# cyh-0/CAVP

Hardware: AMD Instinct MI355X
Metric: frames/sec end-to-end CAVP fwd+bwd, B=32 224x224 (higher is better)
Workload: dtype bf16; 1 GPU; C1' (config_avss_binary shape): CAVP ResNet-50 OS16 + VGGish, training step = forward_train (batch-stat BN, 32 images + 64 audio clips per GPU) + cross-entropy + full backward, 224x224 RGB + 96x64 mel, num_classes=2, random-init (synthetic) weights; global_batch=32, per_gpu_batch=32, parallelism=dp1, ranks=1, launch=hipGraph replay, deterministic=False

## Files before the change

cavp_amd/csrc/conv_igemm_big.hip:

```cpp
#include <type_traits>

#include "igemm_params.h"

#define CAVP_USE8(a) asm volatile("" : "+v"(a[0]), "+v"(a[1]), "+v"(a[2]), "+v"(a[3]), "+v"(a[4]), "+v"(a[5]), "+v"(a[6]), "+v"(a[7]))

namespace {

constexpr int BC = 256, BP = 256, NT = 512;
constexpr int HALF_BYTES = 128 * 128;
constexpr int BUF_BYTES = 4 * HALF_BYTES;
constexpr int RING_BYTES = 2 * BUF_BYTES;
constexpr int SCR_BYTES = 4096;
constexpr int LDS_BYTES = RING_BYTES + 8 * SCR_BYTES;
constexpr unsigned kOOB = 0x80000000u;
static_assert(LDS_BYTES == 160 * 1024, "the whole LDS of a CU");

typedef __attribute__((address_space(3))) void* lds_ptr_t;

}

template <int DBG>
__global__ __launch_bounds__(512, 2) void igemm_big_kernel(const IgemmParams p) {
  extern __shared__ __attribute__((aligned(16))) char smem[];
  cavp_prefetch_kernargs<(int)sizeof(IgemmParams)>();
  const int tid = threadIdx.x, lane = tid & 63;
  const int wave = __builtin_amdgcn_readfirstlane(tid >> 6);
  const int wc = wave & 3, wp = wave >> 2;
  const int lrow = lane & 15, lgrp = lane >> 4;

  const __amdgpu_buffer_rsrc_t xrsrc = __builtin_amdgcn_make_buffer_rsrc((void*)p.x, 0, p.x_bytes, 0x00020000);
  const __amdgpu_buffer_rsrc_t wrsrc = __builtin_amdgcn_make_buffer_rsrc((void*)p.w, 0, p.w_bytes, 0x00020000);

  const int my_tiles = ((int)blockIdx.x < p.nblk) ? (p.nblk - 1 - (int)blockIdx.x) / (int)gridDim.x + 1 : 0;
  if (my_tiles == 0) return;
  const int HoWo = p.Ho * p.Wo;

  const int r0 = 8 * wave + (lane >> 3);
  const int kslot = ((lane & 7) ^ ((4 * wave + (lane >> 4)) & 7)) * 8;
  const int kbyte = kslot * 2;
  unsigned w_off[4];
  unsigned x_off[4];
  unsigned x_mask[4];
  int iss_tile = 0;
  int iss_ti = 0, iss_cc = 0;
  int iss_buf = 0;
  int iss_woff = p.tap_woff[0], iss_xoff = p.tap_xoff[0];

  auto setup_tile = [&](int ord) {
    const int vb = (int)blockIdx.x + ord * (int)gridDim.x;
    const int sid = xcd_remap(vb, p.nblk);
    const int tp = fast_div(sid, p.div_tc_m, p.div_tc_s), tc = sid - tp * p.tiles_c;
    const int c_base = tc * BC, p_base = tp * BP;
#pragma unroll
    for (int m = 0; m < 4; ++m) {
      const int r = r0 + 64 * (m & 1), half = m >> 1;
      const int c = c_base + (r >> 5) * 64 + half * 32 + (r & 31);
      w_off[m] = c < p.Cout ? (unsigned)(((size_t)c * p.K + kslot) * 2) : kOOB;
    }
    int h0[4], w0[4];
#pragma unroll
    for (int m = 0; m < 4; ++m) {
      const int r = r0 + 64 * (m & 1), half = m >> 1;
      const int pix = p_base + (r >> 6) * 128 + half * 64 + (r & 63);
      const bool ok = pix < p.M;
      const int pp = ok ? pix : 0;
      const int n = fast_div(pp, p.div_hw_m, p.div_hw_s), rr = pp - n * HoWo;
      const int ho = fast_div(rr, p.div_w_m, p.div_w_s), wo = rr - ho * p.Wo;
      h0[m] = ok ? ho * p.stride - p.pad : -0x10000000;
      w0[m] = wo * p.stride_w - p.pad;
      x_mask[m] = 0;
      x_off[m] = (unsigned)((n * p.H + h0[m]) * p.W + w0[m]) * (unsigned)(p.ldx * 2) + (unsigned)kbyte;
    }
    for (int t = 0; t < p.ntaps; ++t) {
      const int dh = p.tap_dh[t], dw = p.tap_dw[t];
#pragma unroll
      for (int m = 0; m < 4; ++m)
        x_mask[m] |= ((unsigned)(h0[m] + dh) < (unsigned)p.H && (unsigned)(w0[m] + dw) < (unsigned)p.W) ? (1u << t) : 0u;
    }
  };

  auto issue_half = [&](auto kc) {
    constexpr int K = decltype(kc)::value;
    const bool live = iss_tile < my_tiles;
    const int ti = iss_ti, c0 = iss_cc * 64;
    const unsigned oobm = (live && (c0 + kslot) < p.Cin) ? 0u : kOOB;
    char* base = smem + iss_buf * BUF_BYTES + K * HALF_BYTES + wave * 1024;
    if constexpr ((DBG & 8) != 0) {
    } else if constexpr ((K & 1) == 0) {
      const unsigned wk = (unsigned)(iss_woff + c0 * 2);
#pragma unroll
      for (int j = 0; j < 2; ++j) {
        const unsigned off = (w_off[(K >> 1) * 2 + j] + wk) | oobm;
        __builtin_amdgcn_raw_ptr_buffer_load_lds(wrsrc, (lds_ptr_t)(base + j * 8192), 16, (int)off, 0, 0, 0);
      }
    } else {
      const unsigned xk = (unsigned)(iss_xoff + c0 * 2);
#pragma unroll
      for (int j = 0; j < 2; ++j) {
        const int m = (K >> 1) * 2 + j;
        const unsigned tapm = ((~(x_mask[m] >> ti)) & 1u) << 31;
        __builtin_amdgcn_raw_ptr_buffer_load_lds(xrsrc, (lds_ptr_t)(base + j * 8192), 16, (int)((x_off[m] + xk) | tapm | oobm), 0, 0,
                                                 0);
      }
    }
    if constexpr (K == 3) {
      iss_buf ^= 1;
      if (live) {
        if constexpr ((DBG & 1) != 0) {
          if (++iss_cc == p.cpt) {
            iss_cc = 0;
            if (++iss_ti == p.ntaps) {
              iss_ti = 0;
              if (++iss_tile < my_tiles) setup_tile(iss_tile);
            }
            iss_woff = p.tap_woff[iss_ti];
            iss_xoff = p.tap_xoff[iss_ti];
          }
        } else {
          if (++iss_ti == p.ntaps) {
            iss_ti = 0;
            if (++iss_cc == p.cpt) {
              iss_cc = 0;
              if (++iss_tile < my_tiles) setup_tile(iss_tile);
            }
          }
          iss_woff = p.tap_woff[iss_ti];
          iss_xoff = p.tap_xoff[iss_ti];
        }
      }
    }
  };

  f32x4_t acc[4][8];
#pragma unroll
  for (int a = 0; a < 4; ++a)
#pragma unroll
    for (int b = 0; b < 8; ++b) acc[a][b] = (f32x4_t){0.f, 0.f, 0.f, 0.f};
  u32x4_t fa0[2][2], fa1[2][2], fb[4][2];

  const int key = (lrow >> 1) & 7;
  const int a_off = (wc * 32 + lrow) * 128 + ((lgrp ^ key) << 4);
  const int b_off = (wp * 64 + lrow) * 128 + ((lgrp ^ key) << 4);
  int cmp_buf = 0, cmp_k = 0, cmp_tile = 0;

  auto read_a = [&](u32x4_t (&f)[2][2], int half) {
    const char* base = smem + cmp_buf * BUF_BYTES + (half ? 2 : 0) * HALF_BYTES + a_off;
#pragma unroll
    for (int a = 0; a < 2; ++a) {
      f[a][0] = *(const u32x4_t*)(base + a * 2048);
      f[a][1] = *(const u32x4_t*)(base + a * 2048 + ((((lgrp ^ key) ^ 4) - (lgrp ^ key)) << 4));
    }
  };
  auto read_b = [&](int half) {
    const char* base = smem + cmp_buf * BUF_BYTES + (half ? 3 : 1) * HALF_BYTES + b_off;
#pragma unroll
    for (int b = 0; b < 4; ++b) {
      fb[b][0] = *(const u32x4_t*)(base + b * 2048);
      fb[b][1] = *(const u32x4_t*)(base + b * 2048 + ((((lgrp ^ key) ^ 4) - (lgrp ^ key)) << 4));
    }
  };
  auto mma_quadrant = [&](const u32x4_t (&f)[2][2], auto hc, auto hq) {
    constexpr int HC = decltype(hc)::value, HQ = decltype(hq)::value;
#pragma unroll
    for (int j = 0; j < 2; ++j)
#pragma unroll
      for (int a = 0; a < 2; ++a)
#pragma unroll
        for (int b = 0; b < 4; ++b) Mma<bf16_t>::run(acc[HC * 2 + a][HQ * 4 + b], f[a][j], fb[b][j]);
  };

  auto epilogue = [&](int ord) {
    const int vb = (int)blockIdx.x + ord * (int)gridDim.x;
    const int sid = xcd_remap(vb, p.nblk);
    const int tp = fast_div(sid, p.div_tc_m, p.div_tc_s), tc = sid - tp * p.tiles_c;
    const int c_wave = tc * BC + wc * 64, p_wave = tp * BP + wp * 128;
    const int nvw = p.M - p_wave;
    if (p.tile_stats) {
#pragma unroll
      for (int a = 0; a < 4; ++a) {
        float s1[4], s2[4], x0[4];
#pragma unroll
        for (int i = 0; i < 4; ++i) {
          x0[i] = row16_first(acc[a][0][i]);
          s1[i] = 0.f; s2[i] = 0.f;
        }
#pragma unroll
        for (int b = 0; b < 8; ++b) {
          const bool ok = b * 16 + lrow < nvw;
#pragma unroll
          for (int i = 0; i < 4; ++i) {
            const float d = ok ? acc[a][b][i] - x0[i] : 0.f;
            s1[i] += d;
            s2[i] = fmaf(d, d, s2[i]);
          }
        }
#pragma unroll
        for (int i = 0; i < 4; ++i) {
          s1[i] = row16_sum(s1[i]);
          s2[i] = row16_sum(s2[i]);
        }
        const int c = c_wave + a * 16 + lgrp * 4;
        if (lrow == 0 && nvw > 0 && c < p.Cout) {
          const float inv_n = fast_rcp((float)(nvw < 128 ? nvw : 128));
          float4 o;
          float m = s1[0] * inv_n; o.x = x0[0] + m; o.y = fmaxf(s2[0] - s1[0] * m, 0.f);
          m = s1[1] * inv_n; o.z = x0[1] + m; o.w = fmaxf(s2[1] - s1[1] * m, 0.f);
          float4 o2;
          m = s1[2] * inv_n; o2.x = x0[2] + m; o2.y = fmaxf(s2[2] - s1[2] * m, 0.f);
          m = s1[3] * inv_n; o2.z = x0[3] + m; o2.w = fmaxf(s2[3] - s1[3] * m, 0.f);
          float* dst = p.tile_stats + ((size_t)(tp * 2 + wp) * p.Cout + c) * 2;
          *(float4*)dst = o;
          *(float4*)(dst + 4) = o2;
        }
      }
    }
    float* scr = (float*)(smem + RING_BYTES + wave * SCR_BYTES);
    const int cg = lane & 7, ec = c_wave + cg * 8, pr = lane >> 3;
    const bool ec_ok = ec < p.Cout;
    float sc[8], sh[8];
#pragma unroll
    for (int e = 0; e < 8; ++e) { sc[e] = 1.f; sh[e] = 0.f; }
    if (ec_ok) {
      if (p.scale) {
#pragma unroll
        for (int q = 0; q < 2; ++q) {
          const float4 t = *(const float4*)(p.scale + ec + 4 * q);
          sc[4 * q] = t.x; sc[4 * q + 1] = t.y; sc[4 * q + 2] = t.z; sc[4 * q + 3] = t.w;
        }
        CAVP_USE8(sc);
      }
      if (p.shift) {
#pragma unroll
        for (int q = 0; q < 2; ++q) {
          const float4 t = *(const float4*)(p.shift + ec + 4 * q);
          sh[4 * q] = t.x; sh[4 * q + 1] = t.y; sh[4 * q + 2] = t.z; sh[4 * q + 3] = t.w;
        }
        CAVP_USE8(sh);
      }
    }
    const bool has_ss = p.scale != nullptr || p.shift != nullptr;
    bf16_t* yp = (bf16_t*)p.y + (size_t)(p_wave + pr) * p.ldy + ec;
    const bf16_t* rp = p.res ? (const bf16_t*)p.res + (size_t)((p.res_rows ? p_wave % p.res_rows : p_wave) + pr) * p.ldr + ec : nullptr;
    bf16_t* xp = p.aux_mode ? (bf16_t*)p.aux + (size_t)(p_wave + pr) * p.ld_aux + ec : nullptr;
#pragma unroll
    for (int b = 0; b < 8; ++b) {
      u32x4_t rr[2], mm[2];
      if (p.aux_mode == 2) {
#pragma unroll
        for (int k = 0; k < 2; ++k) {
          mm[k] = (u32x4_t){0u, 0u, 0u, 0u};
          if (ec_ok && b * 16 + pr + 8 * k < nvw) {
            mm[k] = *(const u32x4_t*)(xp + (size_t)(b * 16 + 8 * k) * p.ld_aux);
            asm volatile("" : "+v"(mm[k]));
          }
        }
      }
      if (rp) {
#pragma unroll
        for (int k = 0; k < 2; ++k) {
          rr[k] = (u32x4_t){0u, 0u, 0u, 0u};
          if (ec_ok && b * 16 + pr + 8 * k < nvw) {
            rr[k] = *(const u32x4_t*)(rp + (size_t)(b * 16 + 8 * k) * p.ldr);
            asm volatile("" : "+v"(rr[k]));
          }
        }
      }
#pragma unroll
      for (int a = 0; a < 4; ++a) *(f32x4_t*)(scr + lrow * 64 + (((a * 4 + lgrp) ^ lrow) << 2)) = acc[a][b];
      __builtin_amdgcn_s_waitcnt(0xc07f);
#pragma unroll
      for (int k = 0; k < 2; ++k) {
        const int px = pr + 8 * k;
        float v[8];
        {
          const f32x4_t t0 = *(const f32x4_t*)(scr + px * 64 + (((2 * cg) ^ px) << 2));
          const f32x4_t t1 = *(const f32x4_t*)(scr + px * 64 + (((2 * cg + 1) ^ px) << 2));
          v[0] = t0[0]; v[1] = t0[1]; v[2] = t0[2]; v[3] = t0[3];
          v[4] = t1[0]; v[5] = t1[1]; v[6] = t1[2]; v[7] = t1[3];
        }
        const int row = b * 16 + px;
        if (!(ec_ok && row < nvw)) continue;
        if (p.nbias) {
          const float* nb = p.nbias + (size_t)fast_div(p_wave + row, p.div_hw_m, p.div_hw_s) * p.Cout + ec;
          float nbv[8];
#pragma unroll
          for (int e = 0; e < 8; ++e) nbv[e] = nb[e];
          CAVP_USE8(nbv);
#pragma unroll
          for (int e = 0; e < 8; ++e) v[e] += nbv[e];
        }
        if (has_ss) {
#pragma unroll
          for (int e = 0; e < 8; ++e) v[e] = __fadd_rn(__fmul_rn(v[e], sc[e]), sh[e]);
        }
        if (p.aux_mode == 2) {
#pragma unroll
          for (int e = 0; e < 4; ++e) {
            v[2 * e] *= __uint_as_float(mm[k][e] << 16);
            v[2 * e + 1] *= __uint_as_float(mm[k][e] & 0xffff0000u);
          }
        }
        if (rp) {
#pragma unroll
          for (int e = 0; e < 4; ++e) {
            v[2 * e] += __uint_as_float(rr[k][e] << 16);
            v[2 * e + 1] += __uint_as_float(rr[k][e] & 0xffff0000u);
          }
        }
        if (p.aux_mode == 1) {
          float dgv[8];
#pragma unroll
          for (int e = 0; e < 8; ++e) gelu_and_grad(v[e], v[e], dgv[e]);
          u32x4_t d;
#pragma unroll
          for (int e = 0; e < 4; ++e) d[e] = pack2bf(dgv[2 * e], dgv[2 * e + 1]);
          __builtin_nontemporal_store(d, (u32x4_t*)(xp + (size_t)(b * 16 + 8 * k) * p.ld_aux));
        } else {
          apply_act_vec<8, true>(v, p.act);
        }
        u32x4_t o;
#pragma unroll
        for (int e = 0; e < 4; ++e) o[e] = pack2bf(v[2 * e], v[2 * e + 1]);
        __builtin_nontemporal_store(o, (u32x4_t*)(yp + (size_t)(b * 16 + 8 * k) * p.ldy));
      }
      __builtin_amdgcn_s_waitcnt(0xc07f);
    }
#pragma unroll
    for (int a = 0; a < 4; ++a)
#pragma unroll
      for (int b = 0; b < 8; ++b) acc[a][b] = (f32x4_t){0.f, 0.f, 0.f, 0.f};
  };

  setup_tile(0);
  const int total_k = my_tiles * p.iters;
  issue_half(std::integral_constant<int, 0>{});
  issue_half(std::integral_constant<int, 1>{});
  issue_half(std::integral_constant<int, 2>{});
  issue_half(std::integral_constant<int, 3>{});
  for (int u = 0; u < total_k; ++u) {
    __builtin_amdgcn_s_waitcnt(vmcnt_imm(0));
    __builtin_amdgcn_s_barrier();
    issue_half(std::integral_constant<int, 0>{});
    issue_half(std::integral_constant<int, 1>{});
    issue_half(std::integral_constant<int, 2>{});
    issue_half(std::integral_constant<int, 3>{});
    if constexpr (!(DBG & 32)) { read_b(0); read_a(fa0, 0); }
    if constexpr (!(DBG & 16)) mma_quadrant(fa0, std::integral_constant<int, 0>{}, std::integral_constant<int, 0>{});
    if constexpr (!(DBG & 32)) read_a(fa1, 1);
    if constexpr (!(DBG & 16)) mma_quadrant(fa1, std::integral_constant<int, 1>{}, std::integral_constant<int, 0>{});
    if constexpr (!(DBG & 32)) read_b(1);
    if constexpr (!(DBG & 16)) {
      mma_quadrant(fa1, std::integral_constant<int, 1>{}, std::integral_constant<int, 1>{});
      mma_quadrant(fa0, std::integral_constant<int, 0>{}, std::integral_constant<int, 1>{});
    }
    cmp_buf ^= 1;
    if (++cmp_k == p.iters) {
      cmp_k = 0;
      if constexpr (!(DBG & 64)) epilogue(cmp_tile);
      ++cmp_tile;
    }
  }
}

template <int DBG>
static hipError_t launch_big(const IgemmParams& p, int nblk, hipStream_t s) {
  static bool attr_set = false;
  if (!attr_set) {
    (void)hipFuncSetAttribute((const void*)igemm_big_kernel<DBG>, hipFuncAttributeMaxDynamicSharedMemorySize, LDS_BYTES);
    attr_set = true;
  }
  IgemmParams q = p;
  q.nblk = nblk;
  const int grid = nblk > 256 ? 256 : nblk;
  igemm_big_kernel<DBG><<<dim3(grid), dim3(NT), LDS_BYTES, s>>>(q);
  return hipGetLastError();
}

hipError_t cavp_launch_igemm_big(const IgemmParams& p, int nblk, hipStream_t s) {
  switch (p.dbg) {
    case 0: return launch_big<0>(p, nblk, s);
#ifdef CAVP_PROFILE
    case 1: return launch_big<1>(p, nblk, s);
    case 8: return launch_big<8>(p, nblk, s);
    case 16: return launch_big<16>(p, nblk, s);
    case 32: return launch_big<32>(p, nblk, s);
    case 64: return launch_big<64>(p, nblk, s);
    case 72: return launch_big<72>(p, nblk, s);
    case 120: return launch_big<120>(p, nblk, s);
#endif
    default: return hipErrorInvalidValue;
  }
}
```

Baseline: 2361 frames/s.

## Software-pipeline epilogue residual/aux loads with explicit vmcnt waits in big igemm

Moves the residual, aux-mask and scale/shift loads in the big implicit-GEMM epilogue to inline-asm global loads. The loads for row block b+1 are issued while block b is processed, using a double-buffered register set and explicit s_waitcnt vmcnt counts. The goal is to hide global load latency behind the LDS transpose and the stores, where before each block loaded its operands and then waited. The vmcnt arithmetic relies on assumptions about how many stores are in flight, so it is fragile. The extra live registers could also hurt occupancy at 2 waves/SIMD.

```diff
diff --git a/cavp_amd/csrc/conv_igemm_big.hip b/cavp_amd/csrc/conv_igemm_big.hip
--- a/cavp_amd/csrc/conv_igemm_big.hip
+++ b/cavp_amd/csrc/conv_igemm_big.hip
@@ -3,6 +3,24 @@
 #include "igemm_params.h"
 
 #define CAVP_USE8(a) asm volatile("" : "+v"(a[0]), "+v"(a[1]), "+v"(a[2]), "+v"(a[3]), "+v"(a[4]), "+v"(a[5]), "+v"(a[6]), "+v"(a[7]))
+
+#define CAVP_VMWAIT(n) asm volatile("s_waitcnt vmcnt(%0)" ::"n"(n) : "memory")
+__device__ __forceinline__ void vm_wait(int n) {
+  switch (n) {
+    case 2: CAVP_VMWAIT(2); break;
+    case 4: CAVP_VMWAIT(4); break;
+    case 6: CAVP_VMWAIT(6); break;
+    default: CAVP_VMWAIT(0); break;
+  }
+}
+template <typename T>
+__device__ __forceinline__ void vm_load16(T& dst, const void* src) {
+  asm volatile("global_load_dwordx4 %0, %1, off" : "=&v"(dst) : "v"(src) : "memory");
+}
+template <typename T>
+__device__ __forceinline__ void vm_load16_hi(T& dst, const void* src) {
+  asm volatile("global_load_dwordx4 %0, %1, off offset:16" : "=&v"(dst) : "v"(src) : "memory");
+}
 
 namespace {
 
@@ -175,6 +193,25 @@
     const int tp = fast_div(sid, p.div_tc_m, p.div_tc_s), tc = sid - tp * p.tiles_c;
     const int c_wave = tc * BC + wc * 64, p_wave = tp * BP + wp * 128;
     const int nvw = p.M - p_wave;
+    float* scr = (float*)(smem + RING_BYTES + wave * SCR_BYTES);
+    const int cg = lane & 7, ec = c_wave + cg * 8, pr = lane >> 3;
+    const bool ec_ok = ec < p.Cout;
+    const bool has_ss = p.scale != nullptr || p.shift != nullptr;
+    bf16_t* yp = (bf16_t*)p.y + (size_t)(p_wave + pr) * p.ldy + ec;
+    const bf16_t* rp = p.res ? (const bf16_t*)p.res + (size_t)((p.res_rows ? p_wave % p.res_rows : p_wave) + pr) * p.ldr + ec : nullptr;
+    bf16_t* xp = p.aux_mode ? (bf16_t*)p.aux + (size_t)(p_wave + pr) * p.ld_aux + ec : nullptr;
+    const bool has_res = p.res != nullptr;
+    const int nl = (p.aux_mode == 2 ? 2 : 0) + (has_res ? 2 : 0);
+    const int ns = (c_wave < p.Cout && nvw >= 128) ? (p.aux_mode == 1 ? 4 : 2) : 0;
+    u32x4_t mm[2][2], rr[2][2];
+    auto issue_operands = [&](int b) {
+#pragma unroll
+      for (int k = 0; k < 2; ++k) {
+        const bool ok = ec_ok && b * 16 + pr + 8 * k < nvw;
+        if (p.aux_mode == 2) vm_load16(mm[b & 1][k], ok ? (const void*)(xp + (size_t)(b * 16 + 8 * k) * p.ld_aux) : p.aux);
+        if (has_res) vm_load16(rr[b & 1][k], ok ? (const void*)(rp + (size_t)(b * 16 + 8 * k) * p.ldr) : p.res);
+      }
+    };
     if (p.tile_stats) {
 #pragma unroll
       for (int a = 0; a < 4; ++a) {
@@ -214,59 +251,35 @@
         }
       }
     }
-    float* scr = (float*)(smem + RING_BYTES + wave * SCR_BYTES);
-    const int cg = lane & 7, ec = c_wave + cg * 8, pr = lane >> 3;
-    const bool ec_ok = ec < p.Cout;
+    f32x4_t scv[2] = {(f32x4_t){1.f, 1.f, 1.f, 1.f}, (f32x4_t){1.f, 1.f, 1.f, 1.f}};
+    f32x4_t shv[2] = {(f32x4_t){0.f, 0.f, 0.f, 0.f}, (f32x4_t){0.f, 0.f, 0.f, 0.f}};
+    if (p.scale) {
+      const float* a = p.scale + (ec_ok ? ec : 0);
+      vm_load16(scv[0], a);
+      vm_load16_hi(scv[1], a);
+    }
+    if (p.shift) {
+      const float* a = p.shift + (ec_ok ? ec : 0);
+      vm_load16(shv[0], a);
+      vm_load16_hi(shv[1], a);
+    }
+    issue_operands(0);
     float sc[8], sh[8];
 #pragma unroll
-    for (int e = 0; e < 8; ++e) { sc[e] = 1.f; sh[e] = 0.f; }
-    if (ec_ok) {
-      if (p.scale) {
-#pragma unroll
-        for (int q = 0; q < 2; ++q) {
-          const float4 t = *(const float4*)(p.scale + ec + 4 * q);
-          sc[4 * q] = t.x; sc[4 * q + 1] = t.y; sc[4 * q + 2] = t.z; sc[4 * q + 3] = t.w;
-        }
-        CAVP_USE8(sc);
-      }
-      if (p.shift) {
-#pragma unroll
-        for (int q = 0; q < 2; ++q) {
-          const float4 t = *(const float4*)(p.shift + ec + 4 * q);
-          sh[4 * q] = t.x; sh[4 * q + 1] = t.y; sh[4 * q + 2] = t.z; sh[4 * q + 3] = t.w;
-        }
-        CAVP_USE8(sh);
-      }
-    }
-    const bool has_ss = p.scale != nullptr || p.shift != nullptr;
-    bf16_t* yp = (bf16_t*)p.y + (size_t)(p_wave + pr) * p.ldy + ec;
-    const bf16_t* rp = p.res ? (const bf16_t*)p.res + (size_t)((p.res_rows ? p_wave % p.res_rows : p_wave) + pr) * p.ldr + ec : nullptr;
-    bf16_t* xp = p.aux_mode ? (bf16_t*)p.aux + (size_t)(p_wave + pr) * p.ld_aux + ec : nullptr;
-#pragma unroll
     for (int b = 0; b < 8; ++b) {
-      u32x4_t rr[2], mm[2];
-      if (p.aux_mode == 2) {
-#pragma unroll
-        for (int k = 0; k < 2; ++k) {
-          mm[k] = (u32x4_t){0u, 0u, 0u, 0u};
-          if (ec_ok && b * 16 + pr + 8 * k < nvw) {
-            mm[k] = *(const u32x4_t*)(xp + (size_t)(b * 16 + 8 * k) * p.ld_aux);
-            asm volatile("" : "+v"(mm[k]));
-          }
-        }
-      }
-      if (rp) {
-#pragma unroll
-        for (int k = 0; k < 2; ++k) {
-          rr[k] = (u32x4_t){0u, 0u, 0u, 0u};
-          if (ec_ok && b * 16 + pr + 8 * k < nvw) {
-            rr[k] = *(const u32x4_t*)(rp + (size_t)(b * 16 + 8 * k) * p.ldr);
-            asm volatile("" : "+v"(rr[k]));
-          }
-        }
-      }
 #pragma unroll
       for (int a = 0; a < 4; ++a) *(f32x4_t*)(scr + lrow * 64 + (((a * 4 + lgrp) ^ lrow) << 2)) = acc[a][b];
+      if (b < 7) issue_operands(b + 1);
+      if (nl || (b == 0 && has_ss)) {
+        vm_wait((b > 0 ? ns : 0) + (b < 7 ? nl : 0));
+        if (p.aux_mode == 2) asm volatile("" : "+v"(mm[b & 1][0]), "+v"(mm[b & 1][1]));
+        if (has_res) asm volatile("" : "+v"(rr[b & 1][0]), "+v"(rr[b & 1][1]));
+      }
+      if (b == 0) {
+        if (has_ss) asm volatile("" : "+v"(scv[0]), "+v"(scv[1]), "+v"(shv[0]), "+v"(shv[1]));
+#pragma unroll
+        for (int e = 0; e < 8; ++e) { sc[e] = scv[e >> 2][e & 3]; sh[e] = shv[e >> 2][e & 3]; }
+      }
       __builtin_amdgcn_s_waitcnt(0xc07f);
 #pragma unroll
       for (int k = 0; k < 2; ++k) {
@@ -296,15 +309,15 @@
         if (p.aux_mode == 2) {
 #pragma unroll
           for (int e = 0; e < 4; ++e) {
-            v[2 * e] *= __uint_as_float(mm[k][e] << 16);
-            v[2 * e + 1] *= __uint_as_float(mm[k][e] & 0xffff0000u);
+            v[2 * e] *= __uint_as_float(mm[b & 1][k][e] << 16);
+            v[2 * e + 1] *= __uint_as_float(mm[b & 1][k][e] & 0xffff0000u);
           }
         }
-        if (rp) {
+        if (has_res) {
 #pragma unroll
           for (int e = 0; e < 4; ++e) {
-            v[2 * e] += __uint_as_float(rr[k][e] << 16);
-            v[2 * e + 1] += __uint_as_float(rr[k][e] & 0xffff0000u);
+            v[2 * e] += __uint_as_float(rr[b & 1][k][e] << 16);
+            v[2 * e + 1] += __uint_as_float(rr[b & 1][k][e] & 0xffff0000u);
           }
         }
         if (p.aux_mode == 1) {
```

After: 2382 frames/s (median of 6 runs). About the same (+0.9%).
